# GreptimeTeam/greptimedb

Measured on NVIDIA H100. Metric: rate() input samples/sec, higher is better.
Workload: dtype f64

## Files before the change

### greptimedb_b200/csrc/b2p_context.cu

```cuda
#include <cstdarg>
#include <cstdio>
#include <cstdlib>
#include <cstring>
#include <new>
#include <string>

#include "b2p_runtime.cuh"

using namespace b2p;

namespace {
thread_local std::string g_err;
}

int fail(int code, const char* fmt, ...) {
  char buf[512];
  va_list ap;
  va_start(ap, fmt);
  vsnprintf(buf, sizeof buf, fmt, ap);
  va_end(ap);
  g_err = buf;
  return code;
}

// ... 24 lines not shown
  cudaError_t e = cudaGetDeviceCount(&ndev);
  if (e != cudaSuccess || ndev == 0) {
    fail(B2P_E_CUDA, "no CUDA device: %s — libb200promql has no CPU fallback", cudaGetErrorString(e));
    cudaGetLastError();
    return nullptr;
  }
  if (device < 0 || device >= ndev) {
    fail(B2P_E_INVALID, "device %d out of range (have %d)", device, ndev);
    return nullptr;
  }
  b2p_ctx* c = new (std::nothrow) b2p_ctx();
  if (!c) {
    fail(B2P_E_NOMEM, "out of host memory");
    return nullptr;
  }
  c->device = device;
  DeviceGuard g(device);
  cudaDeviceProp prop;
  if (cudaGetDeviceProperties(&prop, device) == cudaSuccess) c->num_sms = prop.multiProcessorCount;
  bool ok = cudaStreamCreateWithFlags(&c->own_stream, cudaStreamNonBlocking) == cudaSuccess;
  c->stream = c->own_stream;
  ok = ok && cudaMalloc(&c->d_ring, kStatusSlots * sizeof(Status)) == cudaSuccess;
  ok = ok && cudaMallocHost(&c->h_ring, kStatusSlots * sizeof(Status)) == cudaSuccess;
  ok = ok && cudaMalloc(&c->d_k0, sizeof(Status)) == cudaSuccess;
  ok = ok && cudaMallocHost(&c->h_k0, sizeof(Status)) == cudaSuccess;
  for (int i = 0; ok && i < 5; ++i)
    for (int j = 0; j < 2; ++j) ok = ok && cudaEventCreate(&c->ev[i][j]) == cudaSuccess;
  if (!ok) {
    fail(B2P_E_CUDA, "context creation failed: %s", cudaGetErrorString(cudaGetLastError()));
    b2p_destroy(c);
    return nullptr;
  }
  cudaMemset(c->d_ring, 0, kStatusSlots * sizeof(Status));
  cudaMemset(c->d_k0, 0, sizeof(Status));
  if (upload_rcp_table() != B2P_OK) {
    b2p_destroy(c);
    return nullptr;
  }
  if (const char* e = getenv("B2P_ENABLE_THREAD_TIER")) c->thread_tier = (e[0] == '1');
  if (const char* e = getenv("B2P_DISABLE_LEAN_TIER")) c->lean_tier = !(e[0] == '1');
  if (const char* e = getenv("B2P_LEAN_ADAPTIVE")) c->lean_adaptive = !(e[0] == '0');
  if (const char* e = getenv("B2P_LEAN_FORCE_FLAGS")) c->lean_force_flags = (e[0] == '1');
  if (const char* e = getenv("B2P_HOST_TS_SCAN")) c->host_ts_scan = (e[0] != '0');
  if (const char* e = getenv("B2P_UNIFORM")) c->uniform_mode = (e[0] == '0') ? 0 : (e[0] == '1' ? 1 : -1);
  if (const char* e = getenv("B2P_COMM_RESERVE_SMS")) c->comm_reserve_sms = atoi(e);
  if (const char* e = getenv("B2P_COMM_HEADSTART_US")) c->comm_headstart_cycles = (long long)(atof(e) * 1980.0);
  if (const char* e = getenv("B2P_ARENA_ROWS")) c->arena_rows_wanted = (size_t)strtoull(e, nullptr, 10);
  return c;
}

void b2p_destroy(b2p_ctx* c) {
  if (!c) return;
  DeviceGuard g(c->device);
  if (c->own_stream) cudaStreamSynchronize(c->own_stream);
  if (c->comm && g_nccl.CommDestroy) g_nccl.CommDestroy(c->comm);
  if (c->s_comm) cudaStreamDestroy(c->s_comm);
  if (c->ev_comm_in) cudaEventDestroy(c->ev_comm_in);
  if (c->ev_comm_done) cudaEventDestroy(c->ev_comm_done);
  if (c->ev_comm_go) cudaEventDestroy(c->ev_comm_go);
  for (int i = 0; i < 5; ++i)
    for (int j = 0; j < 2; ++j)
      if (c->ev[i][j]) cudaEventDestroy(c->ev[i][j]);
  for (int i = 0; i < 2; ++i) {
    if (c->ev_h2d[i]) cudaEventDestroy(c->ev_h2d[i]);
    if (c->ev_comp[i]) cudaEventDestroy(c->ev_comp[i]);
    if (c->ev_d2h[i]) cudaEventDestroy(c->ev_d2h[i]);
  }
  if (c->s_h2d) cudaStreamDestroy(c->s_h2d);
  if (c->s_d2h) cudaStreamDestroy(c->s_d2h);
  if (c->d_ring) cudaFree(c->d_ring);
  if (c->h_ring) cudaFreeHost(c->h_ring);
  if (c->d_k0) cudaFree(c->d_k0);
  if (c->h_k0) cudaFreeHost(c->h_k0);
  if (c->own_stream) cudaStreamDestroy(c->own_stream);
  delete c;
}

int b2p_set_stream(b2p_ctx* c, void* cuda_stream) {
  if (!c) return fail(B2P_E_INVALID, "ctx is NULL");
  c->stream = reinterpret_cast<cudaStream_t>(cuda_stream);
  return B2P_OK;
}

int b2p_use_own_stream(b2p_ctx* c) {
  if (!c) return fail(B2P_E_INVALID, "ctx is NULL");
  c->stream = c->own_stream;
  return B2P_OK;
}

int64_t b2p_last_slow_series(b2p_ctx* c) { return c ? c->last_slow : -1; }
int64_t b2p_last_h2d_bytes(b2p_ctx* c) { return c ? c->last_h2d_bytes : -1; }
int64_t b2p_last_warp_tier_series(b2p_ctx* c) { return c ? c->last_w : -1; }
int64_t b2p_launch_count(b2p_ctx* c) { return c ? c->launches : -1; }

double b2p_last_kernel_ms(b2p_ctx* c, int stage) {
  if (!c || stage < 0 || stage >= 5 || !c->ev_used[stage]) return -1.0;
  DeviceGuard g(c->device);
  float ms = -1.f;
  if (cudaEventElapsedTime(&ms, c->ev[stage][0], c->ev[stage][1]) != cudaSuccess) {
    cudaGetLastError();
    return -1.0;
  }
  return (double)ms;
}


// ... 45 lines not shown
```

### greptimedb_b200/csrc/b2p_range.cu

```cuda
#include <algorithm>
#include <atomic>
#include <cstring>
#include <memory>
#include <string>
#include <thread>
#include <vector>

#include <cub/device/device_scan.cuh>

#include "b2p_runtime.cuh"
#include "b2p_subquery.cuh"
#include "b2p_kernel_t.cuh"
#include "b2p_kernel_lean.cuh"
#include "b2p_kernels.cuh"

using namespace b2p;

namespace {

constexpr int kRing = 256;
constexpr int kBigRing = 1024;
constexpr int kSlowCtas = 132;
constexpr int kSlowWarps = kSlowCtas * 4;
constexpr size_t kArenaDefaultRows = 1u << 21;

void stage_begin_on(b2p_ctx* c, int stage, cudaStream_t s) { cudaEventRecord(c->ev[stage][0], s); }
void stage_end_on(b2p_ctx* c, int stage, cudaStream_t s) {
  cudaEventRecord(c->ev[stage][1], s);
  c->ev_used[stage] = true;
}

constexpr bool rate_like(int fn) { return fn == B2P_FN_RATE || fn == B2P_FN_INCREASE || fn == B2P_FN_DELTA; }

template <int FN, bool TS32>
int launch_fast_t(b2p_ctx* c, const RangeArgs& a) {
  constexpr size_t smem = (size_t)kWarpsPerCta * (2 * kRing * (8 + (TS32 ? 4 : 8)) + kRing / 8) + kRcpTable * 8;
  auto kern = range_fast_kernel<FN, kRing, TS32>;
  unsigned grid = 0;
  if (int rc = persistent_grid(c, kern, smem, kWarpsPerCta, a.n_series, &grid)) return rc;
  if (grid == 0) return B2P_OK;
  kern<<<grid, kWarpsPerCta * 32, smem, c->stream>>>(a);
  c->launches++;
  CU(cudaGetLastError());
  return B2P_OK;
}

template <int FN>
int launch_big(b2p_ctx* c, const RangeArgs& a0) {
  RangeArgs a = a0;
  a.use_w_list = 2;
  constexpr size_t smem = (size_t)kWarpsPerCta * (2 * kBigRing * (8 + 4) + kBigRing / 8) + kRcpTable * 8;
  auto kern = range_fast_kernel<FN, kBigRing, true>;
  unsigned grid = 0;
  if (int rc = persistent_grid(c, kern, smem, kWarpsPerCta, kAllResident, &grid)) return rc;
// ... 630 lines not shown
extern "C" {

int b2p_subquery_dev(b2p_ctx* c, const b2p_range_params* p, int64_t inner_start, int64_t inner_interval,
                     const double* vals, const uint32_t* valid, uint32_t n_rows, uint64_t T_inner, double* out,
                     uint32_t* out_valid) {
  if (!c) return fail(B2P_E_INVALID, "ctx is NULL");
  int64_t T = 0;
  int rc = check_grid(p, n_rows, &T);
  if (rc) return rc;
  if (p->range == 0) return fail(B2P_E_INVALID, "subquery: zero range");
  if (p->offset != 0 || p->filter_nan != 0) return fail(B2P_E_INVALID, "subquery: offset and filter_nan must be 0");
  if (inner_interval <= 0) return fail(B2P_E_INVALID, "subquery: inner interval must be > 0 (got %lld)", (long long)inner_interval);
  if (n_rows == 0 || T == 0) return B2P_OK;
  if (!out || !out_valid || (T_inner && (!vals || !valid))) return fail(B2P_E_INVALID, "NULL argument");
  DeviceGuard g(c->device);
  if (T_inner == 0) {
    CU(cudaMemsetAsync(out, 0, (size_t)n_rows * (size_t)T * 8, c->stream));
    CU(cudaMemsetAsync(out_valid, 0, (size_t)n_rows * (size_t)((T + 31) / 32) * 4, c->stream));
    return B2P_OK;
  }
  return subquery_run(c, p, inner_start, inner_interval, vals, valid, n_rows, T_inner, T, out, out_valid);
}

int b2p_synth_fill_dev(b2p_ctx* c, uint64_t series_begin, uint64_t n_series, uint32_t n_samples, int64_t t0,
                       int64_t scrape_ms, uint32_t jitter_ms, int32_t with_resets, uint64_t seed, int64_t* ts,
                       double* val, uint32_t* sid) {
  if (!c || !ts || !val) return fail(B2P_E_INVALID, "NULL argument");
  DeviceGuard g(c->device);
  const uint64_t total = n_series * (uint64_t)n_samples;
  if (total == 0) return B2P_OK;
  synth_fill_kernel<<<capped_grid(c, total, 256, 32), 256, 0, c->stream>>>(series_begin, n_series, n_samples, t0,
                                                                           scrape_ms, jitter_ms, with_resets, seed, ts,
                                                                           val, sid);
  c->launches++;
  CU(cudaGetLastError());
  return B2P_OK;
}

}

SeriesIn stage_series(Staging& s, const int64_t* ts, const double* val, const uint32_t* sid, uint32_t sid_base,
                      const uint64_t* offsets_host, uint64_t n_rows, uint32_t n_series) {
  SeriesIn in{s.in(ts, n_rows * 8), s.in(val, n_rows * 8), nullptr};
  if (offsets_host) {
    in.offsets = s.in(offsets_host, ((size_t)n_series + 1) * 8);
  } else {
    const uint32_t* d_sid = s.in(sid, n_rows * 4);
    in.offsets = static_cast<uint64_t*>(s.buf(((size_t)n_series + 1) * 8));
    if (!s.rc) s.rc = series_offsets_impl(s.c, d_sid, n_rows, n_series, sid_base, in.offsets);
  }
  return in;
}

extern "C" {

static int host_scan_series(const int64_t* ts, const uint32_t* sid, const uint64_t* offsets_in, uint64_t n_rows,
                            uint32_t n_series, uint32_t sid_base, uint64_t* offsets_out, int64_t* t0, int64_t* cadence,
                            int32_t* all_regular) {
  if (sid) {
    uint64_t r = 0;
    uint32_t prev = sid_base;
    offsets_out[0] = 0;
    uint32_t next = 0;
    for (; r < n_rows; ++r) {
      const uint32_t id = sid[r];
      if (id < prev || id - sid_base >= n_series) return B2P_E_UNSORTED;
      const uint32_t local = id - sid_base;
      while (next < local) offsets_out[++next] = r;
      prev = id;
    }
    while (next < n_series) offsets_out[++next] = n_rows;
  } else {
    for (uint32_t s = 0; s <= n_series; ++s) offsets_out[s] = offsets_in[s] - offsets_in[0];
    for (uint32_t s = 0; s < n_series; ++s)
      if (offsets_out[s + 1] < offsets_out[s] || offsets_out[s + 1] > n_rows) return B2P_E_INVALID;
  }
  bool regular = true;
  for (uint32_t s = 0; s < n_series; ++s) {
    const uint64_t r0 = offsets_out[s], r1 = offsets_out[s + 1];
    const int64_t first = r1 > r0 ? ts[r0] : 0;
    const int64_t step = r1 - r0 >= 2 ? (int64_t)((uint64_t)ts[r0 + 1] - (uint64_t)first) : 0;
    if (t0) t0[s] = first;
    if (cadence) cadence[s] = step;
    if (regular) {
      uint64_t expect = (uint64_t)first;
      for (uint64_t r = r0; r < r1; ++r) {
        if ((uint64_t)ts[r] != expect) { regular = false; break; }
        expect += (uint64_t)step;
      }
    }
    if (!regular && !t0 && !cadence) break;
  }
  if (all_regular) *all_regular = regular ? 1 : 0;
  return B2P_OK;
}

int b2p_host_scan_series(const int64_t* ts, const uint32_t* sid, const uint64_t* offsets_in, uint64_t n_rows,
                         uint32_t n_series, uint32_t sid_base, uint64_t* offsets_out, int64_t* t0, int64_t* cadence,
                         int32_t* all_regular) {
  if (!offsets_out || (!sid && !offsets_in) || (!ts && n_rows)) return fail(B2P_E_INVALID, "NULL argument");
  const int rc = host_scan_series(ts, sid, offsets_in, n_rows, n_series, sid_base, offsets_out, t0, cadence, all_regular);
  if (rc == B2P_E_UNSORTED) return fail(rc, "series-id column is not non-decreasing or out of range");
  if (rc) return fail(rc, "offsets are not non-decreasing or exceed n_rows");
  return rc;
}

static int range_eval_host_simple(b2p_ctx* c, const b2p_range_params* p, const int64_t* ts, const double* val,
                                  const uint32_t* sid, uint32_t sid_base, const uint64_t* offsets_host, uint64_t n_rows,
                                  uint32_t n_series, int64_t T, double* out, uint32_t* valid_words) {
  int rc;
  const uint32_t Tw = (uint32_t)((T + 31) / 32);
  c->last_h2d_bytes = (long long)(n_rows * 16 + (offsets_host ? ((size_t)n_series + 1) * 8 : n_rows * 4));
  Staging s{c};
  const SeriesIn in = stage_series(s, ts, val, sid, sid_base, offsets_host, n_rows, n_series);
  double* d_out = s.out(out, (size_t)n_series * (size_t)T * 8);
  uint32_t* d_valid = s.out(valid_words, (size_t)n_series * Tw * 4);
  if ((rc = s.rc) || (rc = b2p_range_eval_dev(c, p, in.ts, in.val, in.offsets, n_rows, n_series, d_out, d_valid)) ||
      (rc = b2p_sync(c)))
    return rc;
  return s.finish();
}

static uint64_t lower_bound_sid(const uint32_t* sid, uint64_t n, uint64_t key) {
  uint64_t lo = 0, hi = n;
  while (lo < hi) {
    const uint64_t mid = (lo + hi) >> 1;
    if ((uint64_t)sid[mid] < key) lo = mid + 1; else hi = mid;
  }
  return lo;
}

int b2p_range_eval(b2p_ctx* c, const b2p_range_params* p, const int64_t* ts, const double* val, const uint32_t* sid,
                   const uint64_t* offsets_host, uint64_t n_rows, uint32_t n_series, double* out,
                   uint32_t* valid_words, int64_t* out_ts) {
  if (!c) return fail(B2P_E_INVALID, "ctx is NULL");
  int64_t T = 0;
  int rc = check_grid(p, n_series, &T);
  if (rc) return rc;
  if (out_ts)
    for (int64_t k = 0; k < T; ++k) out_ts[k] = p->start + k * p->interval;
  if (n_series == 0 || T == 0) return B2P_OK;
  if (!sid && !offsets_host) return fail(B2P_E_INVALID, "need sid or offsets_host");
  if (!out || !valid_words || ((!ts || !val) && n_rows)) return fail(B2P_E_INVALID, "NULL argument");
  DeviceGuard g(c->device);
  if (!c->pending.empty() && (rc = b2p_sync(c))) return rc;
  const uint32_t Tw = (uint32_t)((T + 31) / 32);

  constexpr uint64_t kChunkRows = 4u << 20;
  if (n_rows <= kChunkRows + kChunkRows / 2 || n_series < 64)
    return range_eval_host_simple(c, p, ts, val, sid, 0u, offsets_host, n_rows, n_series, T, out, valid_words);

  const uint64_t avg_rows = n_rows / n_series + 1;
  uint32_t C = (uint32_t)(kChunkRows / avg_rows);
  if (C < 64) C = 64;
  const uint32_t n_chunks = (n_series + C - 1) / C;
  if (!c->pipe_ready) {
    bool ok = cudaStreamCreateWithFlags(&c->s_h2d, cudaStreamNonBlocking) == cudaSuccess;
    ok = ok && cudaStreamCreateWithFlags(&c->s_d2h, cudaStreamNonBlocking) == cudaSuccess;
    for (int i = 0; ok && i < 2; ++i) {
      ok = ok && cudaEventCreateWithFlags(&c->ev_h2d[i], cudaEventDisableTiming) == cudaSuccess;
      ok = ok && cudaEventCreateWithFlags(&c->ev_comp[i], cudaEventDisableTiming) == cudaSuccess;
      ok = ok && cudaEventCreateWithFlags(&c->ev_d2h[i], cudaEventDisableTiming) == cudaSuccess;
    }
    if (!ok) return fail(B2P_E_CUDA, "pipeline stream/event creation failed");
    c->pipe_ready = true;
  }
  if ((rc = c->p_status.ensure((size_t)n_chunks * sizeof(Status)))) return rc;
  Status* h_stat = nullptr;
  CU(cudaMallocHost(&h_stat, (size_t)n_chunks * sizeof(Status)));
  uint64_t* h_offs[2] = {nullptr, nullptr};
  if (offsets_host) {
    for (int i = 0; i < 2; ++i) CU(cudaMallocHost(&h_offs[i], ((size_t)C + 1) * 8));
  }
  struct Cleanup {
    Status* s; uint64_t* o0; uint64_t* o1;
    ~Cleanup() { if (s) cudaFreeHost(s); if (o0) cudaFreeHost(o0); if (o1) cudaFreeHost(o1); }
  } cleanup{h_stat, h_offs[0], h_offs[1]};

  uint64_t max_rows = 0;
  std::vector<uint64_t> chunk_row(n_chunks + 1, 0);
  {
    uint64_t prev = 0;
    for (uint32_t i = 0; i < n_chunks; ++i) {
      const uint64_t s1 = (uint64_t)(i + 1) * C < n_series ? (uint64_t)(i + 1) * C : n_series;
      const uint64_t r1 = offsets_host ? offsets_host[s1] : lower_bound_sid(sid, n_rows, s1);
      if (r1 < prev) return fail(B2P_E_UNSORTED, "series-id column is not non-decreasing");
      if (r1 - prev > max_rows) max_rows = r1 - prev;
      prev = r1;
      chunk_row[i + 1] = r1;
    }
    if (!offsets_host && prev != n_rows) return fail(B2P_E_UNSORTED, "series id >= n_series");
  }
  const bool scan = c->host_ts_scan && !offsets_host;
  uint64_t* h_doff = nullptr;
  int64_t *h_t0 = nullptr, *h_cad = nullptr;
  std::unique_ptr<std::atomic<int>[]> scan_state;
  std::atomic<bool> scan_stop{false};
  std::vector<std::thread> scan_workers;
  struct ScanJoin {
    std::atomic<bool>& stop; std::vector<std::thread>& w; uint64_t*& a; int64_t*& b; int64_t*& d;
    ~ScanJoin() {
      stop.store(true);
      for (auto& t : w) if (t.joinable()) t.join();
      if (a) cudaFreeHost(a);
      if (b) cudaFreeHost(b);
      if (d) cudaFreeHost(d);
    }
  } scan_join{scan_stop, scan_workers, h_doff, h_t0, h_cad};
  if (scan) {
    CU(cudaMallocHost(&h_doff, ((size_t)n_series + n_chunks) * 8));
    CU(cudaMallocHost(&h_t0, (size_t)n_series * 8));
    CU(cudaMallocHost(&h_cad, (size_t)n_series * 8));
    scan_state.reset(new std::atomic<int>[n_chunks]);
    for (uint32_t i = 0; i < n_chunks; ++i) scan_state[i].store(0);
    unsigned hw = std::thread::hardware_concurrency();
    unsigned W = hw >= 64 ? 16u : (hw >= 8 ? hw / 4 : 1u);
    if (W > n_chunks) W = n_chunks;
    std::atomic<int>* state = scan_state.get();
    const uint64_t* rows = chunk_row.data();
    try {
    for (unsigned k = 0; k < W; ++k) {
      scan_workers.emplace_back([=, &scan_stop]() {
        for (uint32_t i = k; i < n_chunks && !scan_stop.load(std::memory_order_relaxed); i += W) {
          const uint32_t s0 = i * C;
          const uint32_t s1 = (uint64_t)s0 + C < n_series ? s0 + C : n_series;
          const uint64_t r0 = rows[i], nr = rows[i + 1] - rows[i];
          int32_t regular = 0;
          const int rc_scan = host_scan_series(ts + r0, sid ? sid + r0 : nullptr, offsets_host ? offsets_host + s0 : nullptr, nr,
                                               s1 - s0, s0, h_doff + s0 + i, h_t0 + s0, h_cad + s0, &regular);
          state[i].store((rc_scan == B2P_OK && regular) ? 1 : 2, std::memory_order_release);
        }
      });
    }
    } catch (...) {
      scan_stop.store(true);
      for (auto& t : scan_workers) if (t.joinable()) t.join();
      for (uint32_t i = 0; i < n_chunks; ++i) {
        int zero = 0;
        state[i].compare_exchange_strong(zero, 2);
      }
    }
  }
  for (int i = 0; i < 2; ++i) {
    if (scan && (rc = c->p_t0[i].ensure((size_t)C * 8))) return rc;
    if (scan && (rc = c->p_cad[i].ensure((size_t)C * 8))) return rc;
    if ((rc = c->p_ts[i].ensure(max_rows * 8 + 16))) return rc;
    if ((rc = c->p_val[i].ensure(max_rows * 8 + 16))) return rc;
    if (!offsets_host && (rc = c->p_sid[i].ensure(max_rows * 4 + 16))) return rc;
    if ((rc = c->p_off[i].ensure(((size_t)C + 1) * 8))) return rc;
    if ((rc = c->p_out[i].ensure((size_t)C * (size_t)T * 8))) return rc;
    if ((rc = c->p_valid[i].ensure((size_t)C * Tw * 4))) return rc;
  }
  CU(cudaStreamSynchronize(c->stream));
  c->last_h2d_bytes = 0;
  uint64_t row_lo = 0;
  for (uint32_t i = 0; i < n_chunks; ++i) {
    const int b = (int)(i & 1);
    const uint32_t s0 = i * C;
    const uint32_t s1 = (uint64_t)s0 + C < n_series ? s0 + C : n_series;
    const uint32_t ns = s1 - s0;
    const uint64_t row_hi = offsets_host ? offsets_host[s1] : lower_bound_sid(sid, n_rows, s1);
    const uint64_t nr = row_hi - row_lo;
    int described = 2;
    if (scan)
      while ((described = scan_state[i].load(std::memory_order_acquire)) == 0) std::this_thread::yield();
    if (i >= 2) CU(cudaStreamWaitEvent(c->s_h2d, c->ev_comp[b], 0));
    CU(cudaMemcpyAsync(c->p_val[b].p, val + row_lo, nr * 8, cudaMemcpyHostToDevice, c->s_h2d));
    c->last_h2d_bytes += (long long)(nr * 8);
    if (described == 1) {
      c->last_h2d_bytes += (long long)(((size_t)ns + 1) * 8 + (size_t)ns * 16);
      CU(cudaMemcpyAsync(c->p_off[b].p, h_doff + s0 + i, ((size_t)ns + 1) * 8, cudaMemcpyHostToDevice, c->s_h2d));
      CU(cudaMemcpyAsync(c->p_t0[b].p, h_t0 + s0, (size_t)ns * 8, cudaMemcpyHostToDevice, c->s_h2d));
      CU(cudaMemcpyAsync(c->p_cad[b].p, h_cad + s0, (size_t)ns * 8, cudaMemcpyHostToDevice, c->s_h2d));
    } else {
    c->last_h2d_bytes += (long long)(nr * 8 + (offsets_host ? ((size_t)ns + 1) * 8 : nr * 4));
    CU(cudaMemcpyAsync(c->p_ts[b].p, ts + row_lo, nr * 8, cudaMemcpyHostToDevice, c->s_h2d));
    if (offsets_host) {
      if (i >= 2) CU(cudaEventSynchronize(c->ev_h2d[b]));
      for (uint32_t q = 0; q <= ns; ++q) h_offs[b][q] = offsets_host[s0 + q] - row_lo;
      CU(cudaMemcpyAsync(c->p_off[b].p, h_offs[b], ((size_t)ns + 1) * 8, cudaMemcpyHostToDevice, c->s_h2d));
    } else {
      CU(cudaMemcpyAsync(c->p_sid[b].p, sid + row_lo, nr * 4, cudaMemcpyHostToDevice, c->s_h2d));
    }
    }
    CU(cudaEventRecord(c->ev_h2d[b], c->s_h2d));
    CU(cudaStreamWaitEvent(c->stream, c->ev_h2d[b], 0));
    if (i >= 2) CU(cudaStreamWaitEvent(c->stream, c->ev_d2h[b], 0));
    if (described == 1) {
      ts_expand_kernel<<<capped_grid(c, ns, 8, 8), 256, 0, c->stream>>>(
          c->p_off[b].as<uint64_t>(), c->p_t0[b].as<int64_t>(), c->p_cad[b].as<int64_t>(), ns, c->p_ts[b].as<int64_t>());
      c->launches++;
      CU(cudaGetLastError());
    } else if (!offsets_host &&
        (rc = series_offsets_impl(c, c->p_sid[b].as<uint32_t>(), nr, ns, s0, c->p_off[b].as<uint64_t>())))
      return rc;
    if ((rc = b2p_range_eval_dev(c, p, c->p_ts[b].as<int64_t>(), c->p_val[b].as<double>(), c->p_off[b].as<uint64_t>(),
                                 nr, ns, c->p_out[b].as<double>(), c->p_valid[b].as<uint32_t>())))
      return rc;
    {
      const int slot = c->pending.back().slot;
      c->pending.pop_back();
      CU(cudaMemcpyAsync(c->p_status.as<Status>() + i, c->d_ring + slot, sizeof(Status), cudaMemcpyDeviceToDevice, c->stream));
    }
    CU(cudaEventRecord(c->ev_comp[b], c->stream));
    CU(cudaStreamWaitEvent(c->s_d2h, c->ev_comp[b], 0));
    CU(cudaMemcpyAsync(out + (size_t)s0 * (size_t)T, c->p_out[b].p, (size_t)ns * (size_t)T * 8, cudaMemcpyDeviceToHost,
                       c->s_d2h));
    CU(cudaMemcpyAsync(valid_words + (size_t)s0 * Tw, c->p_valid[b].p, (size_t)ns * Tw * 4, cudaMemcpyDeviceToHost,
                       c->s_d2h));
    CU(cudaEventRecord(c->ev_d2h[b], c->s_d2h));
    row_lo = row_hi;
  }
  CU(cudaMemcpyAsync(h_stat, c->p_status.p, (size_t)n_chunks * sizeof(Status), cudaMemcpyDeviceToHost, c->stream));
  CU(cudaMemcpyAsync(c->h_k0, c->d_k0, sizeof(Status), cudaMemcpyDeviceToHost, c->stream));
  CU(cudaStreamSynchronize(c->stream));
  CU(cudaStreamSynchronize(c->s_d2h));
  if (const uint32_t k0 = c->h_k0->k0_errors) {
    CU(cudaMemsetAsync(c->d_k0, 0, sizeof(Status), c->stream));
// ... 105 lines not shown
```

### greptimedb_b200/csrc/b2p_runtime.cuh

```cuda
#pragma once
#include <cuda_runtime.h>
#include <dlfcn.h>

#include <cstdint>
#include <cstdlib>
#include <map>
#include <string>
#include <type_traits>
#include <utility>
#include <vector>

#include "../../include/b200promql.h"
#include "b2p_status.cuh"

int fail(int code, const char* fmt, ...);

#define CU(x)                                                                                   \
  do {                                                                                          \
    cudaError_t e__ = (x);                                                                      \
    if (e__ != cudaSuccess) return fail(B2P_E_CUDA, "%s: %s (%s:%d)", #x, cudaGetErrorString(e__), __FILE__, __LINE__); \
  } while (0)

int k0_fail(uint32_t k0);

struct Nccl {
  typedef struct ncclComm* comm_t;
  struct unique_id { char internal[128]; };
  enum { kSum = 0, kMax = 2, kMin = 3 };
  enum { kUint32 = 3, kInt64 = 4, kUint64 = 5, kFloat64 = 8 };
  int (*GetUniqueId)(unique_id*) = nullptr;
  int (*CommInitRank)(comm_t*, int, unique_id, int) = nullptr;
  int (*CommDestroy)(comm_t) = nullptr;
  int (*AllReduce)(const void*, void*, size_t, int, int, comm_t, cudaStream_t) = nullptr;
  int (*GroupStart)() = nullptr;
  int (*GroupEnd)() = nullptr;
  const char* (*GetErrorString)(int) = nullptr;
  void* handle = nullptr;
  bool load() {
    if (handle) return true;
    const char* names[] = {getenv("B2P_NCCL_LIB"), "libnccl.so.2", "libnccl.so"};
    for (const char* n : names) {
      if (!n || !*n) continue;
      handle = dlopen(n, RTLD_NOW | RTLD_GLOBAL);
      if (handle) break;
    }
    if (!handle) return false;
    bool ok = true;
    auto sym = [&](const char* n) { void* p = dlsym(handle, n); ok = ok && p; return p; };
    GetUniqueId = reinterpret_cast<decltype(GetUniqueId)>(sym("ncclGetUniqueId"));
    CommInitRank = reinterpret_cast<decltype(CommInitRank)>(sym("ncclCommInitRank"));
    CommDestroy = reinterpret_cast<decltype(CommDestroy)>(sym("ncclCommDestroy"));
    AllReduce = reinterpret_cast<decltype(AllReduce)>(sym("ncclAllReduce"));
    GroupStart = reinterpret_cast<decltype(GroupStart)>(sym("ncclGroupStart"));
    GroupEnd = reinterpret_cast<decltype(GroupEnd)>(sym("ncclGroupEnd"));
    GetErrorString = reinterpret_cast<decltype(GetErrorString)>(sym("ncclGetErrorString"));
    if (!ok) { handle = nullptr; }
    return ok;
  }
};
extern Nccl g_nccl;

#define NCCL_TRY(x)                                                                                          \
  do {                                                                                                       \
    int r__ = (x);                                                                                           \
    if (r__ != 0) return fail(B2P_E_CUDA, "%s: %s", #x, g_nccl.GetErrorString ? g_nccl.GetErrorString(r__) : "NCCL error"); \
  } while (0)

struct DevBuf {
  void* p = nullptr;
  size_t cap = 0;
  DevBuf() = default;
  DevBuf(DevBuf&& o) noexcept : p(o.p), cap(o.cap) { o.p = nullptr; o.cap = 0; }
  DevBuf(const DevBuf&) = delete;
  DevBuf& operator=(const DevBuf&) = delete;
  ~DevBuf() {
    if (p) cudaFree(p);
  }
  int ensure(size_t bytes) {
    if (bytes <= cap) return B2P_OK;
    if (p) cudaFree(p);
    p = nullptr;
    cap = 0;
    size_t want = bytes + bytes / 8 + 256;
    cudaError_t e = cudaMalloc(&p, want);
    if (e != cudaSuccess) {
      e = cudaMalloc(&p, bytes);
      want = bytes;
    }
    if (e != cudaSuccess) {
      cudaGetLastError();
      return fail(B2P_E_NOMEM, "cudaMalloc(%zu) failed: %s", bytes, cudaGetErrorString(e));
    }
    cap = want;
    return B2P_OK;
  }
  template <class T>
  T* as() const { return reinterpret_cast<T*>(p); }
};

constexpr int kStatusSlots = 32;
constexpr int kStageSlots = 11;

struct b2p_group_index {
  uint32_t n_series = 0, n_groups = 0;
  uint32_t max_members = 0;
  uint32_t* gid = nullptr;
  uint32_t* goff = nullptr;
  uint32_t* members = nullptr;
  std::vector<uint32_t> goff_host;
};

struct b2p_ctx {
  int device = 0;
  int num_sms = 132;
  cudaStream_t own_stream = nullptr, stream = nullptr;
  b2p::Status* d_ring = nullptr;
  b2p::Status* h_ring = nullptr;
  b2p::Status* d_k0 = nullptr;
  b2p::Status* h_k0 = nullptr;
  int next_slot = 0;
  struct Pending {
    int slot; int fn; b2p::RangeArgs args; int lean_mode; bool thread_tier; bool used_lean; uint32_t n_series; bool verdict_taken;
    bool fused;
    bool merged;
  };
  std::vector<Pending> pending;
  DevBuf slow_list, w_list, b_list, arena_ts, arena_val, win_scratch;
  Nccl::comm_t comm = nullptr;
  int comm_ranks = 1, comm_rank = 0;
  long long comm_headstart_cycles = 60000;
  int comm_reserve_sms = 0;
  int comm_reserve_now = 0;
  cudaStream_t s_comm = nullptr;
  cudaEvent_t ev_comm_in = nullptr, ev_comm_done = nullptr, ev_comm_go = nullptr;
  DevBuf m_tmp0, m_tmp1;
  DevBuf w_skip, b_skip, slow_skip;
  bool fused_pending = false;
  bool thread_tier = false;
  bool lean_tier = true;
  bool lean_force_flags = false;
  bool lean_adaptive = true;
  int lean_mode[B2P_FN__COUNT] = {};
  int lean_backoff[B2P_FN__COUNT] = {};
  int last_lean_mode = 0;
  int last_range_fn = 0;
  bool last_used_lean = false;
  uint32_t last_range_series = 0;
  int uniform_mode = -1;
  size_t arena_rows = 0;
  size_t arena_rows_wanted = 0;
  cudaEvent_t ev[5][2] = {};
  bool ev_used[5] = {false, false, false, false, false};
  long long launches = 0;
  long long last_slow = 0;
  long long last_w = 0;
  DevBuf stage[kStageSlots];
  bool pipe_ready = false;
  cudaStream_t s_h2d = nullptr, s_d2h = nullptr;
  cudaEvent_t ev_h2d[2] = {}, ev_comp[2] = {}, ev_d2h[2] = {};
  DevBuf p_ts[2], p_val[2], p_sid[2], p_off[2], p_out[2], p_valid[2], p_status;
  DevBuf p_t0[2], p_cad[2];
  bool host_ts_scan = true;
  long long last_h2d_bytes = 0;
  DevBuf hq_off, hq_series, hq_les;
  DevBuf rg_out, rg_valid;
  DevBuf g_keys_in, g_keys_out, g_vals_in, g_vals_out, g_goff, g_tmp;
  DevBuf c_psum, c_pcnt;
  DevBuf s_goff[2], s_members[2], s_mask;
  DevBuf sc_state;
  DevBuf t_table, t_cand, t_state;
  DevBuf q_table, q_state, q_hist;
  DevBuf v_keys, v_alt, v_rank, v_seg, v_group, v_tmp;
  DevBuf sq_ts, sq_val, sq_off, sq_tmp;
  DevBuf so_off, so_keys, so_cells, so_tmp;
  std::map<std::pair<const void*, size_t>, int> blocks_per_sm;
};

struct DeviceGuard {
  int prev = -1;
  explicit DeviceGuard(int dev) {
    cudaGetDevice(&prev);
    if (prev != dev) cudaSetDevice(dev);
  }
  ~DeviceGuard() {
    int cur = -1;
    cudaGetDevice(&cur);
    if (prev >= 0 && cur != prev) cudaSetDevice(prev);
  }
};

inline void stage_begin(b2p_ctx* c, int stage) {
  cudaEventRecord(c->ev[stage][0], c->stream);
}
inline void stage_end(b2p_ctx* c, int stage) {
  cudaEventRecord(c->ev[stage][1], c->stream);
  c->ev_used[stage] = true;
}

inline unsigned capped_grid(const b2p_ctx* c, uint64_t units, uint64_t per_block, uint64_t per_sm) {
  const uint64_t blocks = (units + per_block - 1) / per_block, cap = (uint64_t)c->num_sms * per_sm;
  return (unsigned)(blocks < cap ? blocks : cap);
}

constexpr uint64_t kAllResident = ~0ull;

template <class Kern>
int persistent_grid(b2p_ctx* c, Kern* kern, size_t smem, int warps, uint64_t units, unsigned* grid) {
  int& per_sm = c->blocks_per_sm[{reinterpret_cast<const void*>(kern), smem}];
  if (per_sm == 0) {
    cudaFuncAttributes fa;
    int nb = 0;
    CU(cudaFuncGetAttributes(&fa, kern));
    if ((size_t)fa.maxDynamicSharedSizeBytes < smem)
      CU(cudaFuncSetAttribute(kern, cudaFuncAttributeMaxDynamicSharedMemorySize, (int)smem));
    CU(cudaOccupancyMaxActiveBlocksPerMultiprocessor(&nb, kern, warps * 32, smem));
// ... 89 lines not shown
```

Before: 99.39 billion.

## Use persistent host scan pool, cached pinned buffers, and piece-level work stealing

Replaces per-call thread spawning and per-call cudaMallocHost of staging buffers with a persistent thread pool and context-cached pinned buffers. Host timestamp regularity scanning is split into fixed-size pieces that workers pull dynamically, and the main thread also pulls pieces while it waits. If the previous chunk's H2D copy has already completed, the main thread sends the chunk without a regularity description. The offsets path now also gets the scan. The aim is to remove pinned-allocation and thread-creation overhead and keep the copy pipeline fed. In exchange it adds locking and condition-variable traffic plus more complex scheduling.

```diff
diff --git a/greptimedb_b200/csrc/b2p_context.cu b/greptimedb_b200/csrc/b2p_context.cu
--- a/greptimedb_b200/csrc/b2p_context.cu
+++ b/greptimedb_b200/csrc/b2p_context.cu
@@ -100,6 +100,7 @@
 void b2p_destroy(b2p_ctx* c) {
   if (!c) return;
   DeviceGuard g(c->device);
+  c->scan_pool.reset();
   if (c->own_stream) cudaStreamSynchronize(c->own_stream);
   if (c->comm && g_nccl.CommDestroy) g_nccl.CommDestroy(c->comm);
   if (c->s_comm) cudaStreamDestroy(c->s_comm);
diff --git a/greptimedb_b200/csrc/b2p_range.cu b/greptimedb_b200/csrc/b2p_range.cu
--- a/greptimedb_b200/csrc/b2p_range.cu
+++ b/greptimedb_b200/csrc/b2p_range.cu
@@ -1,5 +1,8 @@
+#include <sched.h>
+
 #include <algorithm>
 #include <atomic>
+#include <chrono>
 #include <cstring>
 #include <memory>
 #include <string>
@@ -736,57 +739,188 @@
   return in;
 }
 
-extern "C" {
-
-static int host_scan_series(const int64_t* ts, const uint32_t* sid, const uint64_t* offsets_in, uint64_t n_rows,
-                            uint32_t n_series, uint32_t sid_base, uint64_t* offsets_out, int64_t* t0, int64_t* cadence,
-                            int32_t* all_regular) {
+
+ScanPool::ScanPool(unsigned n_threads) {
+  try {
+    for (unsigned k = 0; k < n_threads; ++k) threads_.emplace_back([this] { loop(); });
+  } catch (...) {
+  }
+}
+
+ScanPool::~ScanPool() {
+  {
+    std::lock_guard<std::mutex> l(m_);
+    quit_ = true;
+  }
+  cv_job_.notify_all();
+  for (auto& t : threads_) t.join();
+}
+
+void ScanPool::run(std::function<void()> job) {
+  {
+    std::lock_guard<std::mutex> l(m_);
+    job_ = std::move(job);
+    busy_ = size();
+    ++generation_;
+  }
+  cv_job_.notify_all();
+}
+
+void ScanPool::wait() {
+  std::unique_lock<std::mutex> l(m_);
+  cv_idle_.wait(l, [this] { return busy_ == 0; });
+}
+
+void ScanPool::loop() {
+  uint64_t seen = 0;
+  for (;;) {
+    std::function<void()> job;
+    {
+      std::unique_lock<std::mutex> l(m_);
+      cv_job_.wait(l, [&] { return quit_ || generation_ != seen; });
+      if (quit_) return;
+      seen = generation_;
+      job = job_;
+    }
+    job();
+    std::lock_guard<std::mutex> l(m_);
+    if (--busy_ == 0) cv_idle_.notify_all();
+  }
+}
+
+namespace {
+
+inline bool on_cadence(const int64_t* ts, uint64_t n, uint64_t first, uint64_t step) {
+  uint64_t acc = 0, expect = first;
+  for (uint64_t r = 0; r < n; ++r) {
+    acc |= (uint64_t)ts[r] ^ expect;
+    expect += step;
+  }
+  return acc == 0;
+}
+inline bool all_ids(const uint32_t* sid, uint64_t n, uint32_t id) {
+  uint32_t acc = 0;
+  for (uint64_t r = 0; r < n; ++r) acc |= sid[r] ^ id;
+  return acc == 0;
+}
+
+int scan_series(const int64_t* ts, const uint32_t* sid, const uint64_t* offsets_in, uint64_t n_rows, uint32_t n_series,
+                uint32_t sid_base, uint64_t row_base, uint64_t* offsets_out, int64_t* t0, int64_t* cadence,
+                bool* regular) {
+  bool reg = true;
+  const bool describe = t0 || cadence;
+  auto series = [&](uint32_t k, uint64_t r0, uint64_t r1) {
+    offsets_out[k] = row_base + r0;
+    if (!describe && !reg) return;
+    const uint64_t first = r1 > r0 ? (uint64_t)ts[r0] : 0;
+    const uint64_t step = r1 - r0 >= 2 ? (uint64_t)ts[r0 + 1] - first : 0;
+    if (t0) t0[k] = (int64_t)first;
+    if (cadence) cadence[k] = (int64_t)step;
+    if (reg) reg = on_cadence(ts + r0, r1 - r0, first, step);
+  };
   if (sid) {
-    uint64_t r = 0;
+    uint32_t next = 0;
     uint32_t prev = sid_base;
-    offsets_out[0] = 0;
-    uint32_t next = 0;
-    for (; r < n_rows; ++r) {
+    uint64_t run = 1;
+    for (uint64_t r = 0; r < n_rows;) {
       const uint32_t id = sid[r];
       if (id < prev || id - sid_base >= n_series) return B2P_E_UNSORTED;
+      uint64_t end = r + 1;
+      if (run > 1 && run <= n_rows - r && all_ids(sid + r, run, id)) end = r + run;
+      while (end < n_rows && sid[end] == id) ++end;
       const uint32_t local = id - sid_base;
-      while (next < local) offsets_out[++next] = r;
+      while (next < local) series(next++, r, r);
+      series(next++, r, end);
+      run = end - r;
       prev = id;
-    }
-    while (next < n_series) offsets_out[++next] = n_rows;
+      r = end;
+    }
+    while (next < n_series) series(next++, n_rows, n_rows);
   } else {
-    for (uint32_t s = 0; s <= n_series; ++s) offsets_out[s] = offsets_in[s] - offsets_in[0];
-    for (uint32_t s = 0; s < n_series; ++s)
-      if (offsets_out[s + 1] < offsets_out[s] || offsets_out[s + 1] > n_rows) return B2P_E_INVALID;
-  }
-  bool regular = true;
-  for (uint32_t s = 0; s < n_series; ++s) {
-    const uint64_t r0 = offsets_out[s], r1 = offsets_out[s + 1];
-    const int64_t first = r1 > r0 ? ts[r0] : 0;
-    const int64_t step = r1 - r0 >= 2 ? (int64_t)((uint64_t)ts[r0 + 1] - (uint64_t)first) : 0;
-    if (t0) t0[s] = first;
-    if (cadence) cadence[s] = step;
-    if (regular) {
-      uint64_t expect = (uint64_t)first;
-      for (uint64_t r = r0; r < r1; ++r) {
-        if ((uint64_t)ts[r] != expect) { regular = false; break; }
-        expect += (uint64_t)step;
-      }
-    }
-    if (!regular && !t0 && !cadence) break;
-  }
-  if (all_regular) *all_regular = regular ? 1 : 0;
-  return B2P_OK;
-}
+    const uint64_t base = offsets_in[0];
+    for (uint32_t k = 0; k < n_series; ++k) {
+      const uint64_t r0 = offsets_in[k] - base, r1 = offsets_in[k + 1] - base;
+      if (r1 < r0 || r1 > n_rows) return B2P_E_INVALID;
+      series(k, r0, r1);
+    }
+  }
+  *regular = reg;
+  return B2P_OK;
+}
+
+constexpr unsigned kMaxScanWorkers = 32;
+unsigned scan_worker_count() {
+  unsigned n = 0;
+  cpu_set_t set;
+  if (sched_getaffinity(0, sizeof set, &set) == 0) n = (unsigned)CPU_COUNT(&set);
+  if (n == 0) n = std::thread::hardware_concurrency();
+  n = n > 1 ? n - 1 : 1;
+  return n < kMaxScanWorkers ? n : kMaxScanWorkers;
+}
+
+struct ChunkScan {
+  static constexpr uint64_t kPieceRows = 1u << 18;
+  struct Piece {
+    uint32_t chunk, s0, s1;
+  };
+  std::vector<Piece> pieces;
+  std::unique_ptr<std::atomic<uint32_t>[]> left;
+  std::unique_ptr<std::atomic<bool>[]> bad;
+  std::unique_ptr<std::atomic<bool>[]> as_is;
+  std::vector<int> verdicts;
+  std::function<bool(const Piece&)> scan;
+  std::atomic<size_t> next{0};
+  std::atomic<bool> stop{false};
+  std::mutex m;
+  std::condition_variable cv;
+  ScanPool* pool = nullptr;
+
+  ~ChunkScan() {
+    if (!pool) return;
+    stop.store(true);
+    pool->wait();
+  }
+  bool take() {
+    if (stop.load(std::memory_order_relaxed)) return false;
+    const size_t k = next.fetch_add(1, std::memory_order_relaxed);
+    if (k >= pieces.size()) return false;
+    const Piece& q = pieces[k];
+    const bool ok = !as_is[q.chunk].load(std::memory_order_relaxed) && scan(q);
+    if (!ok) bad[q.chunk].store(true, std::memory_order_relaxed);
+    if (left[q.chunk].fetch_sub(1, std::memory_order_acq_rel) == 1) {
+      std::lock_guard<std::mutex> l(m);
+      verdicts[q.chunk] = bad[q.chunk].load(std::memory_order_relaxed) ? 2 : 1;
+      cv.notify_all();
+    }
+    return true;
+  }
+  bool ready(uint32_t i, int* v) {
+    std::lock_guard<std::mutex> l(m);
+    *v = verdicts[i];
+    return *v != 0;
+  }
+  void send_as_is(uint32_t i) { as_is[i].store(true, std::memory_order_relaxed); }
+  void wait(uint32_t i) {
+    std::unique_lock<std::mutex> l(m);
+    cv.wait_for(l, std::chrono::microseconds(50), [&] { return verdicts[i] != 0; });
+  }
+};
+
+}
+
+extern "C" {
 
 int b2p_host_scan_series(const int64_t* ts, const uint32_t* sid, const uint64_t* offsets_in, uint64_t n_rows,
                          uint32_t n_series, uint32_t sid_base, uint64_t* offsets_out, int64_t* t0, int64_t* cadence,
                          int32_t* all_regular) {
   if (!offsets_out || (!sid && !offsets_in) || (!ts && n_rows)) return fail(B2P_E_INVALID, "NULL argument");
-  const int rc = host_scan_series(ts, sid, offsets_in, n_rows, n_series, sid_base, offsets_out, t0, cadence, all_regular);
+  bool regular = true;
+  const int rc = scan_series(ts, sid, offsets_in, n_rows, n_series, sid_base, 0, offsets_out, t0, cadence, &regular);
   if (rc == B2P_E_UNSORTED) return fail(rc, "series-id column is not non-decreasing or out of range");
   if (rc) return fail(rc, "offsets are not non-decreasing or exceed n_rows");
-  return rc;
+  offsets_out[n_series] = sid ? n_rows : offsets_in[n_series] - offsets_in[0];
+  if (all_regular) *all_regular = regular ? 1 : 0;
+  return B2P_OK;
 }
 
 static int range_eval_host_simple(b2p_ctx* c, const b2p_range_params* p, const int64_t* ts, const double* val,
@@ -850,16 +984,13 @@
     c->pipe_ready = true;
   }
   if ((rc = c->p_status.ensure((size_t)n_chunks * sizeof(Status)))) return rc;
-  Status* h_stat = nullptr;
-  CU(cudaMallocHost(&h_stat, (size_t)n_chunks * sizeof(Status)));
+  if ((rc = c->hp_status.ensure((size_t)n_chunks * sizeof(Status)))) return rc;
+  Status* h_stat = c->hp_status.as<Status>();
   uint64_t* h_offs[2] = {nullptr, nullptr};
-  if (offsets_host) {
-    for (int i = 0; i < 2; ++i) CU(cudaMallocHost(&h_offs[i], ((size_t)C + 1) * 8));
-  }
-  struct Cleanup {
-    Status* s; uint64_t* o0; uint64_t* o1;
-    ~Cleanup() { if (s) cudaFreeHost(s); if (o0) cudaFreeHost(o0); if (o1) cudaFreeHost(o1); }
-  } cleanup{h_stat, h_offs[0], h_offs[1]};
+  for (int i = 0; offsets_host && i < 2; ++i) {
+    if ((rc = c->hp_off[i].ensure(((size_t)C + 1) * 8))) return rc;
+    h_offs[i] = c->hp_off[i].as<uint64_t>();
+  }
 
   uint64_t max_rows = 0;
   std::vector<uint64_t> chunk_row(n_chunks + 1, 0);
@@ -875,55 +1006,61 @@
     }
     if (!offsets_host && prev != n_rows) return fail(B2P_E_UNSORTED, "series id >= n_series");
   }
-  const bool scan = c->host_ts_scan && !offsets_host;
+  ChunkScan cs;
   uint64_t* h_doff = nullptr;
   int64_t *h_t0 = nullptr, *h_cad = nullptr;
-  std::unique_ptr<std::atomic<int>[]> scan_state;
-  std::atomic<bool> scan_stop{false};
-  std::vector<std::thread> scan_workers;
-  struct ScanJoin {
-    std::atomic<bool>& stop; std::vector<std::thread>& w; uint64_t*& a; int64_t*& b; int64_t*& d;
-    ~ScanJoin() {
-      stop.store(true);
-      for (auto& t : w) if (t.joinable()) t.join();
-      if (a) cudaFreeHost(a);
-      if (b) cudaFreeHost(b);
-      if (d) cudaFreeHost(d);
-    }
-  } scan_join{scan_stop, scan_workers, h_doff, h_t0, h_cad};
+  bool scan = c->host_ts_scan;
+  if (scan && !c->scan_pool) c->scan_pool.reset(new (std::nothrow) ScanPool(scan_worker_count()));
+  scan = scan && c->scan_pool && c->scan_pool->size() > 0;
   if (scan) {
-    CU(cudaMallocHost(&h_doff, ((size_t)n_series + n_chunks) * 8));
-    CU(cudaMallocHost(&h_t0, (size_t)n_series * 8));
-    CU(cudaMallocHost(&h_cad, (size_t)n_series * 8));
-    scan_state.reset(new std::atomic<int>[n_chunks]);
-    for (uint32_t i = 0; i < n_chunks; ++i) scan_state[i].store(0);
-    unsigned hw = std::thread::hardware_concurrency();
-    unsigned W = hw >= 64 ? 16u : (hw >= 8 ? hw / 4 : 1u);
-    if (W > n_chunks) W = n_chunks;
-    std::atomic<int>* state = scan_state.get();
+    if ((rc = c->hp_doff.ensure(((size_t)n_series + n_chunks) * 8)) || (rc = c->hp_t0.ensure((size_t)n_series * 8)) ||
+        (rc = c->hp_cad.ensure((size_t)n_series * 8)))
+      return rc;
+    h_doff = c->hp_doff.as<uint64_t>();
+    h_t0 = c->hp_t0.as<int64_t>();
+    h_cad = c->hp_cad.as<int64_t>();
+    cs.left.reset(new std::atomic<uint32_t>[n_chunks]);
+    cs.bad.reset(new std::atomic<bool>[n_chunks]);
+    cs.as_is.reset(new std::atomic<bool>[n_chunks]);
+    cs.verdicts.assign(n_chunks, 0);
+    const uint32_t per_piece = (uint32_t)std::max<uint64_t>(1, ChunkScan::kPieceRows / avg_rows);
+    for (uint32_t i = 0; i < n_chunks; ++i) {
+      const uint32_t s0 = i * C;
+      const uint32_t s1 = (uint64_t)s0 + C < n_series ? s0 + C : n_series;
+      const uint64_t r0 = chunk_row[i], r1 = chunk_row[i + 1];
+      h_doff[s1 + i] = r1 - r0;
+      cs.bad[i].store(false);
+      cs.as_is[i].store(false);
+      if (offsets_host && ((i == 0 && offsets_host[0] != 0) || r1 > n_rows)) {
+        cs.left[i].store(0);
+        cs.verdicts[i] = 2;
+        continue;
+      }
+      uint32_t n_pieces = 0;
+      for (uint32_t a = s0; a < s1; a = (uint32_t)std::min<uint64_t>((uint64_t)a + per_piece, s1), ++n_pieces)
+        cs.pieces.push_back({i, a, (uint32_t)std::min<uint64_t>((uint64_t)a + per_piece, s1)});
+      cs.left[i].store(n_pieces);
+    }
     const uint64_t* rows = chunk_row.data();
-    try {
-    for (unsigned k = 0; k < W; ++k) {
-      scan_workers.emplace_back([=, &scan_stop]() {
-        for (uint32_t i = k; i < n_chunks && !scan_stop.load(std::memory_order_relaxed); i += W) {
-          const uint32_t s0 = i * C;
-          const uint32_t s1 = (uint64_t)s0 + C < n_series ? s0 + C : n_series;
-          const uint64_t r0 = rows[i], nr = rows[i + 1] - rows[i];
-          int32_t regular = 0;
-          const int rc_scan = host_scan_series(ts + r0, sid ? sid + r0 : nullptr, offsets_host ? offsets_host + s0 : nullptr, nr,
-                                               s1 - s0, s0, h_doff + s0 + i, h_t0 + s0, h_cad + s0, &regular);
-          state[i].store((rc_scan == B2P_OK && regular) ? 1 : 2, std::memory_order_release);
-        }
-      });
-    }
-    } catch (...) {
-      scan_stop.store(true);
-      for (auto& t : scan_workers) if (t.joinable()) t.join();
-      for (uint32_t i = 0; i < n_chunks; ++i) {
-        int zero = 0;
-        state[i].compare_exchange_strong(zero, 2);
-      }
-    }
+    cs.scan = [=](const ChunkScan::Piece& q) {
+      const uint64_t r0 = rows[q.chunk], r1 = rows[q.chunk + 1];
+      auto first_row = [&](uint32_t s) -> uint64_t {
+        if (s == q.chunk * C) return r0;
+        if (s == std::min<uint64_t>((uint64_t)q.chunk * C + C, n_series)) return r1;
+        return offsets_host ? offsets_host[s] : r0 + lower_bound_sid(sid + r0, r1 - r0, s);
+      };
+      const uint64_t ra = first_row(q.s0), rb = first_row(q.s1);
+      if (!(r0 <= ra && ra <= rb && rb <= r1)) return false;
+      bool regular = false;
+      return scan_series(ts + ra, sid ? sid + ra : nullptr, offsets_host ? offsets_host + q.s0 : nullptr, rb - ra,
+                         q.s1 - q.s0, q.s0, ra - r0, h_doff + q.s0 + q.chunk, h_t0 + q.s0, h_cad + q.s0,
+                         &regular) == B2P_OK && regular;
+    };
+    ChunkScan* job = &cs;
+    cs.pool = c->scan_pool.get();
+    cs.pool->run([job]() {
+      while (job->take()) {}
+    });
   }
   for (int i = 0; i < 2; ++i) {
     if (scan && (rc = c->p_t0[i].ensure((size_t)C * 8))) return rc;
@@ -946,8 +1083,14 @@
     const uint64_t row_hi = offsets_host ? offsets_host[s1] : lower_bound_sid(sid, n_rows, s1);
     const uint64_t nr = row_hi - row_lo;
     int described = 2;
-    if (scan)
-      while ((described = scan_state[i].load(std::memory_order_acquire)) == 0) std::this_thread::yield();
+    while (scan && !cs.ready(i, &described)) {
+      if (i >= 1 && cudaEventQuery(c->ev_h2d[i >= 2 ? b : 0]) == cudaSuccess) {
+        cs.send_as_is(i);
+        described = 2;
+        break;
+      }
+      if (!cs.take()) cs.wait(i);
+    }
     if (i >= 2) CU(cudaStreamWaitEvent(c->s_h2d, c->ev_comp[b], 0));
     CU(cudaMemcpyAsync(c->p_val[b].p, val + row_lo, nr * 8, cudaMemcpyHostToDevice, c->s_h2d));
     c->last_h2d_bytes += (long long)(nr * 8);
diff --git a/greptimedb_b200/csrc/b2p_runtime.cuh b/greptimedb_b200/csrc/b2p_runtime.cuh
--- a/greptimedb_b200/csrc/b2p_runtime.cuh
+++ b/greptimedb_b200/csrc/b2p_runtime.cuh
@@ -2,10 +2,15 @@
 #include <cuda_runtime.h>
 #include <dlfcn.h>
 
+#include <condition_variable>
 #include <cstdint>
 #include <cstdlib>
+#include <functional>
 #include <map>
+#include <memory>
+#include <mutex>
 #include <string>
+#include <thread>
 #include <type_traits>
 #include <utility>
 #include <vector>
@@ -96,6 +101,53 @@
   }
   template <class T>
   T* as() const { return reinterpret_cast<T*>(p); }
+};
+
+struct HostBuf {
+  void* p = nullptr;
+  size_t cap = 0;
+  HostBuf() = default;
+  HostBuf(const HostBuf&) = delete;
+  HostBuf& operator=(const HostBuf&) = delete;
+  ~HostBuf() {
+    if (p) cudaFreeHost(p);
+  }
+  int ensure(size_t bytes) {
+    if (bytes <= cap) return B2P_OK;
+    if (p) cudaFreeHost(p);
+    p = nullptr;
+    cap = 0;
+    const size_t want = bytes + bytes / 8 + 256;
+    const cudaError_t e = cudaMallocHost(&p, want);
+    if (e != cudaSuccess) {
+      p = nullptr;
+      cudaGetLastError();
+      return fail(B2P_E_NOMEM, "cudaMallocHost(%zu) failed: %s", want, cudaGetErrorString(e));
+    }
+    cap = want;
+    return B2P_OK;
+  }
+  template <class T>
+  T* as() const { return reinterpret_cast<T*>(p); }
+};
+
+class ScanPool {
+ public:
+  explicit ScanPool(unsigned n_threads);
+  ~ScanPool();
+  unsigned size() const { return (unsigned)threads_.size(); }
+  void run(std::function<void()> job);
+  void wait();
+
+ private:
+  void loop();
+  std::vector<std::thread> threads_;
+  std::mutex m_;
+  std::condition_variable cv_job_, cv_idle_;
+  std::function<void()> job_;
+  uint64_t generation_ = 0;
+  unsigned busy_ = 0;
+  bool quit_ = false;
 };
 
 constexpr int kStatusSlots = 32;
@@ -161,6 +213,8 @@
   DevBuf p_ts[2], p_val[2], p_sid[2], p_off[2], p_out[2], p_valid[2], p_status;
   DevBuf p_t0[2], p_cad[2];
   bool host_ts_scan = true;
+  HostBuf hp_status, hp_doff, hp_t0, hp_cad, hp_off[2];
+  std::unique_ptr<ScanPool> scan_pool;
   long long last_h2d_bytes = 0;
   DevBuf hq_off, hq_series, hq_les;
   DevBuf rg_out, rg_valid;
diff --git a/profiles/e2e_bench.py b/profiles/e2e_bench.py
--- /dev/null
+++ b/profiles/e2e_bench.py
@@ -0,0 +1,166 @@
+from __future__ import annotations
+
+import argparse
+import ctypes as C
+import json
+import os
+import statistics
+import sys
+import time
+from concurrent.futures import ThreadPoolExecutor
+
+ROOT = os.path.dirname(os.path.dirname(os.path.abspath(__file__)))
+sys.path.insert(0, ROOT)
+sys.path.insert(0, os.path.join(ROOT, "profiles"))
+
+from binary_bench import gpu_identity
+
+N, SCRAPE, T0, RANGE, SEED = 1000, 15_000, 1_700_000_000_000, 300_000, 0x5EED
+CHUNK_ROWS = 4 << 20
+
+
+def chunks(S: int, n_rows: int):
+    C_ = max(64, CHUNK_ROWS // (n_rows // S + 1))
+    return [(s0, min(C_, S - s0), s0 * N, min(C_, S - s0) * N) for s0 in range(0, S, C_)]
+
+
+def link(torch, nbytes: int, copies: int):
+    h_src = torch.empty(nbytes, dtype=torch.uint8).pin_memory()
+    h_dst = torch.empty(nbytes, dtype=torch.uint8).pin_memory()
+    d_in = torch.empty(nbytes, dtype=torch.uint8, device="cuda")
+    d_out = torch.empty(nbytes, dtype=torch.uint8, device="cuda")
+    s1, s2 = torch.cuda.Stream(), torch.cuda.Stream()
+
+    def timed(h2d: bool, d2h: bool) -> float:
+        torch.cuda.synchronize()
+        ev = [torch.cuda.Event(enable_timing=True) for _ in range(2)]
+        ev[0].record()
+        for s in (s1, s2):
+            s.wait_event(ev[0])
+        for _ in range(copies):
+            if h2d:
+                with torch.cuda.stream(s1):
+                    d_in.copy_(h_src, non_blocking=True)
+            if d2h:
+                with torch.cuda.stream(s2):
+                    h_dst.copy_(d_out, non_blocking=True)
+        cur = torch.cuda.current_stream()
+        for s in (s1, s2):
+            cur.wait_stream(s)
+        ev[1].record()
+        torch.cuda.synchronize()
+        return ev[0].elapsed_time(ev[1]) * 1e-3
+
+    timed(True, True)
+    t_h2d, t_d2h, t_both = timed(True, False), timed(False, True), timed(True, True)
+    gb = nbytes * copies / 1e9
+    return {"chunk_bytes": nbytes, "copies": copies, "h2d_alone_GBps": gb / t_h2d, "d2h_alone_GBps": gb / t_d2h,
+            "both_at_once_total_GBps": 2 * gb / t_both}
+
+
+def main():
+    ap = argparse.ArgumentParser()
+    ap.add_argument("--series", type=int, default=131_072)
+    ap.add_argument("--reps", type=int, default=10)
+    ap.add_argument("--copies", type=int, default=32)
+    ap.add_argument("--out", default=None, help="write the result here as JSON (it is printed either way)")
+    args = ap.parse_args()
+    assert args.reps >= 8
+
+    import numpy as np
+    import torch
+    from greptimedb_b200 import Context, _lib, make_params
+
+    assert torch.cuda.is_available(), "e2e_bench needs a CUDA device"
+    S = args.series
+    n_rows, T = S * N, N
+    Tw = (T + 31) // 32
+    res = {"lib": _lib.LIB_PATH, **gpu_identity(), "cpu_count": os.cpu_count(),
+           "cpu_affinity": len(os.sched_getaffinity(0)), "series": S, "rows": n_rows, "T": T}
+
+    ctx = Context(0)
+    ctx.use_torch_stream()
+    ts = torch.empty(n_rows, dtype=torch.int64, device="cuda")
+    val = torch.empty(n_rows, dtype=torch.float64, device="cuda")
+    sid = torch.empty(n_rows, dtype=torch.int32, device="cuda")
+    ctx.synth_fill_dev(0, S, N, T0, SCRAPE, 0, 0, SEED, ts, val, sid)
+    ctx.sync()
+    h_ts, h_val, h_sid = ts.cpu().pin_memory(), val.cpu().pin_memory(), sid.cpu().pin_memory()
+    h_off = (torch.arange(S + 1, dtype=torch.int64) * N).pin_memory()
+    h_out = torch.zeros(S * T, dtype=torch.float64).pin_memory()
+    h_valid = torch.zeros(S * Tw, dtype=torch.int32).pin_memory()
+    del ts, val, sid
+    torch.cuda.synchronize()
+    ctx.use_own_stream()
+
+    ch = chunks(S, n_rows)
+    res["chunks"] = len(ch)
+    res["link"] = link(torch, ch[0][3] * 8, args.copies)
+
+    L = _lib.load()
+    P = lambda t, off=0: C.c_void_p(t.data_ptr() + off * t.element_size())
+
+    def scan(chunk, with_ids: bool):
+        s0, ns, r0, nr = chunk
+        out = np.zeros(ns + 1, np.uint64)
+        t0 = np.zeros(ns, np.int64)
+        cad = np.zeros(ns, np.int64)
+        reg = C.c_int32(-1)
+        p = lambda a: a.ctypes.data_as(C.c_void_p)
+        rc = L.b2p_host_scan_series(P(h_ts, r0), P(h_sid, r0) if with_ids else None, None if with_ids else P(h_off, s0),
+                                    nr, ns, s0, p(out), p(t0), p(cad), C.addressof(reg))
+        assert rc == 0 and reg.value == 1, L.b2p_last_error().decode()
+
+    workers = max(1, len(os.sched_getaffinity(0)) - 1)
+    res["scan"] = {"workers": workers}
+    for route, with_ids, row_bytes in (("ids", True, 12), ("offsets", False, 8)):
+        one = []
+        for _ in range(5):
+            t = time.perf_counter()
+            scan(ch[0], with_ids)
+            one.append(time.perf_counter() - t)
+        t1 = statistics.median(one)
+        with ThreadPoolExecutor(workers) as ex:
+            list(ex.map(lambda c_: scan(c_, with_ids), ch))
+            t = time.perf_counter()
+            list(ex.map(lambda c_: scan(c_, with_ids), ch))
+            tn = time.perf_counter() - t
+        res["scan"][route] = {"one_chunk_one_thread_ms": t1 * 1e3,
+                              "one_thread_GBps": ch[0][3] * row_bytes / t1 / 1e9,
+                              "all_chunks_ms": tn * 1e3, "all_chunks_GBps": n_rows * row_bytes / tn / 1e9,
+                              "all_chunks_rows_per_s": n_rows / tn}
+
+    p = make_params("rate", T0, T0 + (N - 1) * SCRAPE, SCRAPE, RANGE)
+    lk = res["link"]
+    res["call"] = {}
+    for route in ("ids", "offsets"):
+        def call():
+            rc = L.b2p_range_eval(ctx._h, C.byref(p), P(h_ts), P(h_val), None if route == "offsets" else P(h_sid),
+                                  P(h_off) if route == "offsets" else None, n_rows, S, P(h_out), P(h_valid), None)
+            assert rc == 0, L.b2p_last_error().decode()
+
+        for _ in range(2):
+            call()
+        times = []
+        for _ in range(args.reps):
+            t = time.perf_counter()
+            call()
+            times.append(time.perf_counter() - t)
+        med = statistics.median(times)
+        h2d, d2h = ctx.last_h2d_bytes(), S * T * 8 + S * Tw * 4
+        least = (h2d + d2h) / (lk["both_at_once_total_GBps"] * 1e9)
+        res["call"][route] = {"median_ms": med * 1e3, "calls_ms": [x * 1e3 for x in times],
+                              "samples_per_s": n_rows / med, "h2d_bytes": h2d, "d2h_bytes": d2h,
+                              "h2d_GBps": h2d / med / 1e9, "d2h_GBps": d2h / med / 1e9,
+                              "link_bound_ms": least * 1e3, "fraction_of_concurrent_link": least / med}
+    ctx.close()
+    line = json.dumps(res)
+    print(line)
+    if args.out:
+        os.makedirs(os.path.dirname(os.path.abspath(args.out)), exist_ok=True)
+        with open(args.out, "w") as f:
+            f.write(line + "\n")
+
+
+if __name__ == "__main__":
+    main()
```

Result: no change. 99.36 billion, median of 6 (-0.0%).
